# rlangefe/pygemma

Hardware: AMD Instinct MI355X
Metric: SNPs/sec (whole node) at n=10,000 c=5; K-eigendecomp wallclock (higher is better)
Workload: dtype i8x3->i32 MFMA (genotype codes exact, integer accumulation exact; U as 24-bit fixed point per eigenvector in three int8 planes) rotation + f64 Gram/sweeps (f32 rounding points of the reference)

## Files before the change

### include/pygemma_hip.h

```cpp
#ifndef PYGEMMA_HIP_H
#define PYGEMMA_HIP_H
#include <stddef.h>
#include <stdint.h>
#ifdef __cplusplus
extern "C" {
#endif

#define PG_OK 0
#define PG_EINVAL (-22)
#define PG_ENOMEM (-12)
#define PG_EHIP (-5)
#define PG_ENOTSUP (-95)
#define PG_ENODEV (-19)

#define PG_MAX_COVARIATES 30

typedef struct pg_ctx pg_ctx;

const char *pg_last_error(void);
const char *pg_version(void);
int pg_device_count(void);
int pg_ctx_create(int device, pg_ctx **out);
int pg_ctx_create_on_stream(int device, void *hip_stream, pg_ctx **out);
void pg_ctx_destroy(pg_ctx *ctx);
// ... 33 lines not shown
int pg_comm_destroy(pg_comm *comm);
int pg_comm_size(const pg_comm *comm);
int pg_comm_rank(const pg_comm *comm);
int pg_comm_broadcast_dev(pg_comm *comm, void *buf, size_t bytes, int root);
int pg_comm_allgather_dev(pg_comm *comm, const void *send, void *recv, size_t bytes_per_rank);
int pg_comm_allreduce_f64_dev(pg_comm *comm, double *buf, size_t count, int op_max);
int pg_comm_barrier(pg_comm *comm);
int pg_comm_group_start(void);
int pg_comm_group_end(void);

int pg_assoc_dev(pg_ctx *ctx, int64_t n, int c, int64_t p, const float *d, const float *Wr, const float *yr,
                 const float *Xr, int64_t ldx, int grid, float *beta, float *se, float *tau, float *lambda,
                 double *F, double *pval, unsigned long long *stats_dev);

int pg_assoc_set_eval_trace(pg_ctx *ctx, unsigned *trace_dev);
int pg_assoc_warm(pg_ctx *ctx, int64_t n, int c);

int pg_assoc_pheno_dev(pg_ctx *ctx, int64_t n, int c, int64_t p, int t, const float *d, const float *Wr,
                       const float *Yr, int64_t ldy, const float *Xr, int64_t ldx, int grid,
                       float *beta, float *se, float *tau, float *lambda, double *F, double *pval,
                       unsigned long long *stats_dev);
int pg_assoc_pheno_warm(pg_ctx *ctx, int64_t n, int c, int t, int64_t p);

int pg_assoc_lrt_dev(pg_ctx *ctx, int64_t n, int c, int64_t p, const float *d, const float *Wr, const float *yr,
                     const float *Xr, int64_t ldx, int grid, float *beta, float *se, float *tau, float *lambda,
                     double *F, double *pval, double *l_alt, double *l_null, double *D_lrt, double *p_lrt);

int pg_score_null_dev(pg_ctx *ctx, int64_t n, int c, const float *d, const float *Wr, const float *yr, float *lambda0_dev);
int pg_score_dev(pg_ctx *ctx, int64_t n, int c, int64_t p, const float *d, const float *Wr, const float *yr, float lambda0,
                 const float *Xr, int64_t ldx, float *beta, float *se, float *tau, float *lambda, double *F, double *pval);
// ... 78 lines not shown
```

### pygemma_amd/csrc/assoc.hip

```cpp
#include "common.hpp"

#include <cmath>

namespace pg {

constexpr int NLAM = 11;
#ifndef PG_ASSOC_WPB
#define PG_ASSOC_WPB 2
#endif
constexpr int WPB = PG_ASSOC_WPB;
#define PG_MINV 1e-35f
#ifndef PG_FUSE_PQ_MAX
#define PG_FUSE_PQ_MAX 36
#endif
#ifndef PG_FUSE_PQR_MAX
#define PG_FUSE_PQR_MAX 28
#endif
#ifndef PG_PFD
#define PG_PFD 2
#endif
#ifndef PG_CHUNK_MIN_NP
#define PG_CHUNK_MIN_NP 80
#endif
#ifndef PG_SCAN_NV
#define PG_SCAN_NV 96
#endif
#ifndef PG_SWEEP_LDS_MIN_SLOTS
#define PG_SWEEP_LDS_MIN_SLOTS 3
#endif
#ifndef PG_PHENO_SPLIT_XE
#define PG_PHENO_SPLIT_XE 26
#endif
#ifndef PG_WAVES
#define PG_WAVES 2
#endif

__host__ __device__ constexpr size_t assoc_per_wave_bytes(int M, bool sweep_lds, size_t evalout_bytes, int n_vals)
{
    return (((sweep_lds ? (size_t)3 * M * 8 : 0) + (size_t)NLAM * 2 * M * 8 + NLAM * evalout_bytes + 2 * NLAM * 4 + (size_t)n_vals * 4) + 15) & ~(size_t)15;
}

struct AssocParams {
    int n, npad, c, niter, nu, grid, rowf;
    long long p, ldx;
    const float *xr;
    const float *fixed;
    float *htab;
    double *fixg;
    double *t1tab;
    float *ldHtab;
    float lam11[NLAM];
    float logl_c;
    const int *leaf, *node, *level, *chunk;
    int n_leaf, n_level, n_chunk, n_vals;
    float *beta, *se, *tau, *lam;
    double *F;
    unsigned long long *stats;
    unsigned *trace;
    int lrt, nhalf;
    float ml_c;
    float *lalt, *lamalt;
    const double *xbuf;
    int xe, xcol;
};

struct EvalOut { float yPy, yPPy, yPPPy, trP, trPP, ld, Pxx_c, Pyx_c, sh, shh; };

__device__ __forceinline__ float hinv_f32(float lam, float d)
{
    const float x = __fadd_rn(__fmul_rn(lam, d), 1.0f);
    const float r0 = __builtin_amdgcn_rcpf(x);
    float r = __builtin_fmaf(__builtin_fmaf(-x, r0, 1.0f), r0, r0);
    if (__builtin_expect(!(x < 0x1p126f), 0)) r = __fdiv_rn(1.0f, x);
// ... 135 lines not shown
    r = (float)((double)r - ((0.5 * (double)pr.n) * ((2.0 * (double)G2) - (double)__fdiv_rn(__fmul_rn(G1, G1), a))) / (double)a);
    return r;
}

template <int C> struct Shape {
    static constexpr int M = C + 2;
    static constexpr int NP = M * (M + 1) / 2;
    static constexpr int SLOTS = (NP + 63) / 64;
    static constexpr int NV0 = NP < 64 ? NP : 64, NV1 = NP > 64 ? NP - 64 : 0;
    static constexpr int slot_nv(int sl) { return (NP - 64 * sl) < 64 ? (NP - 64 * sl) : 64; }
    static constexpr bool CHUNKED = NP > PG_CHUNK_MIN_NP;
    static constexpr bool SWEEP_LDS = SLOTS >= PG_SWEEP_LDS_MIN_SLOTS;
    static constexpr int SCAN_NV = (M <= 4 && PG_SCAN_NV > 64) ? 64 : PG_SCAN_NV;
    static constexpr int G = (SCAN_NV / (2 * M)) < 1 ? 1 : ((SCAN_NV / (2 * M)) > 11 ? 11 : (SCAN_NV / (2 * M)));
    static constexpr bool FUSE_PQ = NP <= PG_FUSE_PQ_MAX, FUSE_PQR = NP <= PG_FUSE_PQR_MAX;
};
__host__ __device__ constexpr int tri(int r, int c) { return r * (r + 1) / 2 + c; }
__host__ __device__ constexpr int next_pow2(int v) { int p = 1; while (p < v) p <<= 1; return p; }

__device__ __forceinline__ double dmaxf(double a, float b) { return ((double)b > a) ? (double)b : a; }

template <int NVP>
__device__ __forceinline__ double reduce_scatter(double (&v)[NVP], int lane)
{
    static_assert(NVP >= 1 && NVP <= 64 && (NVP & (NVP - 1)) == 0, "power of two");
#pragma unroll
    for (int s = 1; s < NVP; s <<= 1) {
        const bool b = (lane & s) != 0;
#pragma unroll
        for (int m = 0; m < NVP / (2 * s); m++) {
            const double keep = b ? v[2 * m + 1] : v[2 * m];
// ... 34 lines not shown
        }
    }
};

template <int SLOTS>
__device__ __forceinline__ double gather(const double (&X)[SLOTS], int es)
{
    double v = __shfl(X[0], es & 63, 64);
#pragma unroll
    for (int sl = 1; sl < SLOTS; sl++) { const double w = __shfl(X[sl], es & 63, 64); v = ((es >> 6) == sl) ? w : v; }
    return v;
}

__device__ __forceinline__ void wave_lds_sync();

template <int C, bool FULL>
__device__ __forceinline__ void lane_sweeps(double (&P)[Shape<C>::SLOTS], double (&Q)[Shape<C>::SLOTS], double (&R)[Shape<C>::SLOTS],
                                            const Own<C> &own, double t1, double t2, int lane, EvalOut &o, double *piv)
{
    constexpr int M = Shape<C>::M, NP = Shape<C>::NP, SLOTS = Shape<C>::SLOTS;
    constexpr bool VIA_LDS = Shape<C>::SWEEP_LDS;
    if (own.valid[0] && own.e[0] == 0) P[0] = dmaxf(P[0], PG_MINV);
    double trP = t1, trPP = t2, apiv = 1.0;
    for (int i = 1; i < M; i++) {
        const int q = i - 1, eqq = tri(q, q);
        double a, b, e = 0.0;
        double ur[SLOTS], uc[SLOTS], vr[SLOTS], vc[SLOTS], wr[SLOTS], wc[SLOTS];
        bool act[SLOTS];
        if constexpr (VIA_LDS) {
#pragma unroll
            for (int sl = 0; sl < SLOTS; sl++)
                if (own.valid[sl] && own.c[sl] == q) {
                    piv[own.r[sl]] = P[sl]; piv[M + own.r[sl]] = Q[sl];
                    if (FULL) piv[2 * M + own.r[sl]] = R[sl];
                }
            wave_lds_sync();
            a = piv[q]; b = piv[M + q];
            if (FULL) e = piv[2 * M + q];
#pragma unroll
            for (int sl = 0; sl < SLOTS; sl++) {
                act[sl] = own.valid[sl] && own.c[sl] >= i;
                const int rr = act[sl] ? own.r[sl] : q, cc = act[sl] ? own.c[sl] : q;
                ur[sl] = piv[rr]; uc[sl] = piv[cc];
                vr[sl] = piv[M + rr]; vc[sl] = piv[M + cc];
                if (FULL) { wr[sl] = piv[2 * M + rr]; wc[sl] = piv[2 * M + cc]; }
            }
            wave_lds_sync();
        } else {
            a = gather<SLOTS>(P, eqq); b = gather<SLOTS>(Q, eqq);
            e = FULL ? gather<SLOTS>(R, eqq) : 0.0;
#pragma unroll
            for (int sl = 0; sl < SLOTS; sl++) {
                act[sl] = own.valid[sl] && own.c[sl] >= i;
                const int er = act[sl] ? tri(own.r[sl], q) : 0, ec = act[sl] ? tri(own.c[sl], q) : 0;
                ur[sl] = gather<SLOTS>(P, er); uc[sl] = gather<SLOTS>(P, ec);
                vr[sl] = gather<SLOTS>(Q, er); vc[sl] = gather<SLOTS>(Q, ec);
                if (FULL) { wr[sl] = gather<SLOTS>(R, er); wc[sl] = gather<SLOTS>(R, ec); }
            }
        }
        if (lane == q) apiv = a;
        const double a2 = a * a, ia = -1.0 / a, ba2 = b / a2;
        if (FULL) {
            const double ba = b / a;
            trPP = (trPP + ba * ba) - 2 * (e / a);
            const double a3 = a2 * a, b2 = b * b;
            const double cR = (e / a2) - (b2 / a3);
#pragma unroll
            for (int sl = 0; sl < SLOTS; sl++)
                if (act[sl]) {
                    double s1 = fma(cR * uc[sl], ur[sl], R[sl]);
                    double s2 = fma(ia * uc[sl], wr[sl], 0.0); s2 = fma(ia * wc[sl], ur[sl], s2);
                    double s3 = fma(ia * vc[sl], vr[sl], 0.0);
                    double s4 = fma(ba2 * uc[sl], vr[sl], 0.0); s4 = fma(ba2 * vc[sl], ur[sl], s4);
                    double rn = ((s1 + s2) + s3) + s4;
                    if (own.r[sl] == i && own.c[sl] == i) rn = dmaxf(rn, PG_MINV);
                    R[sl] = rn;
                }
        }
        trP = trP - b / a;
#pragma unroll
        for (int sl = 0; sl < SLOTS; sl++)
            if (act[sl]) {
                double s1 = fma(ba2 * uc[sl], ur[sl], Q[sl]);
                double s2 = fma(ia * uc[sl], vr[sl], 0.0); s2 = fma(ia * vc[sl], ur[sl], s2);
                double qn = s1 + s2;
                double pn = fma(ia * uc[sl], ur[sl], P[sl]);
                if (own.r[sl] == i && own.c[sl] == i) { qn = dmaxf(qn, PG_MINV); pn = dmaxf(pn, PG_MINV); }
                Q[sl] = qn; P[sl] = pn;
            }
        if (i == M - 2) { o.Pxx_c = (float)gather<SLOTS>(P, tri(M - 2, M - 2)); o.Pyx_c = (float)gather<SLOTS>(P, tri(M - 1, M - 2)); }
    }
    const double lg = log(apiv);
    float ld = 0.0f;
    for (int q = 0; q < M - 1; q++) ld = (float)((double)ld + __shfl(lg, q, 64));
    o.yPy = (float)gather<SLOTS>(P, NP - 1);
    o.yPPy = (float)gather<SLOTS>(Q, NP - 1);
    o.yPPPy = FULL ? (float)gather<SLOTS>(R, NP - 1) : 0.0f;
    o.trP = (float)trP;
    o.trPP = FULL ? (float)trPP : 0.0f;
    o.ld = ld;
    o.sh = (float)t1;
    o.shh = FULL ? (float)t2 : 0.0f;
}

template <int C> struct Elem {
    static constexpr int S4 = (C + 2 + 3) / 4;
    float4 row[S4];
    float x;
};
template <int C, bool HASX = true>
__device__ __forceinline__ void load_elem(const AssocParams &pr, const float *xrow, int i, Elem<C> &e)
{
    const float4 *src = reinterpret_cast<const float4 *>(pr.fixed + (size_t)i * pr.rowf);
// ... 122 lines not shown
            }
        if constexpr (SL == 0 && PW == 1) s += hd;
        if constexpr (SL == 0 && PW == 3) s = fma(hd, hd, s);
    });
    out = reduce_scatter<NVP>(acc, lane);
    if constexpr (SL == 0 && (PW == 1 || PW == 3)) tsum = bfly(s);
}
template <int C, int PW, bool HASX, int SL = 0, class EL = WaldElem<C>>
__device__ __forceinline__ void slot_passes(const AssocParams &pr, typename EL::Row xrow, float lam, int lane, float *htab_out,
                                            double (&X)[Shape<C>::SLOTS], double &tsum)
{
    gram_pass_slot<C, PW, SL, HASX, EL>(pr, xrow, lam, lane, SL == 0 ? htab_out : nullptr, X[SL], tsum);
    if constexpr (SL + 1 < Shape<C>::SLOTS) slot_passes<C, PW, HASX, SL + 1, EL>(pr, xrow, lam, lane, htab_out, X, tsum);
}

template <int C, bool FULL, class EL = WaldElem<C>>
__device__ __forceinline__ void eval_specific(const AssocParams &pr, typename EL::Row xrow, float lam, int lane, const Own<C> &own, EvalOut &o,
                                              double *piv)
{
    constexpr int SLOTS = Shape<C>::SLOTS;
    double P[SLOTS], Q[SLOTS], R[SLOTS], t1 = 0.0, t2 = 0.0;
#pragma unroll
    for (int sl = 0; sl < SLOTS; sl++) R[sl] = 0.0;
    if constexpr (Shape<C>::CHUNKED) {
        double tq = 0.0;
        slot_passes<C, 1, true, 0, EL>(pr, xrow, lam, lane, nullptr, P, t1);
        slot_passes<C, 2, true, 0, EL>(pr, xrow, lam, lane, nullptr, Q, tq);
        if (FULL) slot_passes<C, 3, true, 0, EL>(pr, xrow, lam, lane, nullptr, R, t2);
    } else if constexpr (FULL && Shape<C>::FUSE_PQR) {
        gram_pass<C, 7, true, EL>(pr, xrow, lam, lane, nullptr, P, Q, R, t1, t2);
    } else if constexpr (Shape<C>::FUSE_PQ) {
        gram_pass<C, 3, true, EL>(pr, xrow, lam, lane, nullptr, P, Q, R, t1, t2);
        if (FULL) gram_pass<C, 4, true, EL>(pr, xrow, lam, lane, nullptr, P, Q, R, t1, t2);
    } else {
        gram_pass<C, 1, true, EL>(pr, xrow, lam, lane, nullptr, P, Q, R, t1, t2);
        gram_pass<C, 2, true, EL>(pr, xrow, lam, lane, nullptr, P, Q, R, t1, t2);
        if (FULL) gram_pass<C, 4, true, EL>(pr, xrow, lam, lane, nullptr, P, Q, R, t1, t2);
    }
    lane_sweeps<C, FULL>(P, Q, R, own, t1, t2, lane, o, piv);
}

template <int C>
__global__ __launch_bounds__(64) void setup_tabs_kernel(AssocParams pr)
{
    constexpr int NP = Shape<C>::NP, SLOTS = Shape<C>::SLOTS;
    extern __shared__ float smem_f[];
    const int t = blockIdx.x, lane = threadIdx.x;
    const float lam = pr.lam11[t];
    Own<C> own;
    own.init(lane);
    double P[SLOTS], Q[SLOTS], R[SLOTS], t1 = 0.0, t2 = 0.0;
    if constexpr (Shape<C>::CHUNKED) {
        double tq = 0.0;
        slot_passes<C, 1, false>(pr, nullptr, lam, lane, pr.htab + (size_t)t * pr.npad, P, t1);
// ... 236 lines not shown
        iteration++;
    }
    return lroot;
}

template <int C, bool LRT, bool PHENO = false>
__global__ __launch_bounds__(64 * WPB, PG_WAVES) void assoc_kernel(AssocParams pr)
{
    constexpr int M = Shape<C>::M, NP = Shape<C>::NP, SLOTS = Shape<C>::SLOTS;
    extern __shared__ unsigned char smem[];
    const int wave = threadIdx.x >> 6, lane = threadIdx.x & 63;
    static_assert(!(PHENO && LRT), "the multi-phenotype search has no LRT");
    const long long g = (long long)blockIdx.x * WPB + wave;
    if (g >= pr.p) return;
    constexpr size_t piv_bytes = Shape<C>::SWEEP_LDS ? (size_t)3 * M * 8 : 0;
    unsigned char *base = smem + (size_t)wave * assoc_per_wave_bytes(M, Shape<C>::SWEEP_LDS, sizeof(EvalOut), pr.n_vals);
    double *piv = reinterpret_cast<double *>(base);
    base += piv_bytes;
    double *xent = reinterpret_cast<double *>(base);
    EvalOut *evs = reinterpret_cast<EvalOut *>(base + (size_t)NLAM * 2 * M * 8);
    float *d1s = reinterpret_cast<float *>(evs + NLAM);
    float *lls = d1s + NLAM;
    float *vals = lls + NLAM;
    const float *xrow = pr.xr + (size_t)g * pr.ldx;

    Own<C> own;
    own.init(lane);
    if constexpr (PHENO) {
        const double *src = pr.xbuf + (size_t)g * NLAM * 2 * pr.xe;
        for (int j = lane; j < NLAM * 2 * M; j += 64) {
            const int tp = j / M, k = j - tp * M;
            xent[j] = src[(size_t)tp * pr.xe + (k <= C ? k : pr.xcol)];
        }
// ... 3 lines not shown
    wave_lds_sync();
    for (int t = 0; t < NLAM; t++) {
        double P[SLOTS], Q[SLOTS], R[SLOTS];
        const double *fp = pr.fixg + ((size_t)t * 2 + 0) * NP, *fq = pr.fixg + ((size_t)t * 2 + 1) * NP;
        const double *xe = xent + t * 2 * M;
#pragma unroll
        for (int sl = 0; sl < SLOTS; sl++) {
            const int r = own.r[sl], c = own.c[sl];
            const bool isx = (r == C) || (r == C + 1 && c == C);
            const int k = (r == C) ? c : C + 1;
            P[sl] = isx ? xe[k] : fp[own.e[sl]];
            Q[sl] = isx ? xe[M + k] : fq[own.e[sl]];
            R[sl] = 0.0;
        }
        EvalOut e;
        lane_sweeps<C, false>(P, Q, R, own, pr.t1tab[t], 0.0, lane, e, piv);
        if (lane == 0) {
            evs[t] = e;
            d1s[t] = d1_f(pr, pr.lam11[t], e.yPy, e.yPPy, e.trP);
            lls[t] = logl_f(pr, e.yPy, pr.ldHtab[t], e.ld);
        }
    }
    wave_lds_sync();
    float best_l = lls[0], best_lambda;
    EvalOut best_e;
    if (best_l < lls[NLAM - 1]) { best_l = lls[NLAM - 1]; best_lambda = pr.lam11[NLAM - 1]; best_e = evs[NLAM - 1]; }
    else { best_lambda = pr.lam11[0]; best_e = evs[0]; }
    unsigned n_fast = 0, n_full = 0;
    if (pr.grid) {
        for (int t = 0; t < NLAM - 1; t++)
            if (lls[t] > best_l) { best_l = lls[t]; best_lambda = pr.lam11[t]; best_e = evs[t]; }
    } else {
        for (int k = 0; k < NLAM - 1; k++) {
            const float f0 = d1s[k], f1 = d1s[k + 1];
            if (__builtin_signbit(f0) == __builtin_signbit(f1)) continue;
            const float l0 = pr.lam11[k], l1 = pr.lam11[k + 1];
            double root = brentq_dev(
                [&](double x) -> double {
                    EvalOut e;
                    const float lf = (float)x;
                    eval_specific<C, false>(pr, xrow, lf, lane, own, e, piv);
                    n_fast++;
                    return (double)d1_f(pr, lf, e.yPy, e.yPPy, e.trP);
                },
                (double)l0, (double)l1, (double)f0, (double)f1);
            const float lroot = newton_dev(pr, (float)root, l0, l1, [&](float lf, EvalOut &e) {
                eval_specific<C, true>(pr, xrow, lf, lane, own, e, piv);
                n_full++;
            });
            EvalOut e;
            eval_specific<C, false>(pr, xrow, lroot, lane, own, e, piv);
            n_fast++;
            const float ldH = device_logdet_H(pr, lroot, lane, vals);
            const float ll = logl_f(pr, e.yPy, ldH, e.ld);
            if (ll > best_l) { best_l = ll; best_lambda = lroot; best_e = e; }
        }
    }
    if constexpr (LRT) {
        float ml_l = ml_logl_f(pr, evs[0].yPy, pr.ldHtab[0]), ml_lam = pr.lam11[0];
        {
            const float l1 = ml_logl_f(pr, evs[NLAM - 1].yPy, pr.ldHtab[NLAM - 1]);
            if (ml_l == ml_l && (l1 != l1 || l1 > ml_l)) { ml_l = l1; ml_lam = pr.lam11[NLAM - 1]; }
        }
        for (int k = 0; k < NLAM - 1; k++) {
            const float f0 = ml_d1_f(pr, pr.lam11[k], evs[k].yPy, evs[k].yPPy, evs[k].sh);
            const float f1 = ml_d1_f(pr, pr.lam11[k + 1], evs[k + 1].yPy, evs[k + 1].yPPy, evs[k + 1].sh);
            if (f0 != f0 || f1 != f1) continue;
            const float s0 = (float)((f0 > 0) - (f0 < 0)), s1 = (float)((f1 > 0) - (f1 < 0));
            if (!(s0 * s1 < 0.0f)) continue;
            double p0 = brentq_dev(
                [&](double x) -> double {
                    EvalOut e;
                    const float lf = (float)x;
                    eval_specific<C, false>(pr, xrow, lf, lane, own, e, piv);
                    n_fast++;
                    return (double)ml_d1_f(pr, lf, e.yPy, e.yPPy, e.sh);
                },
                (double)pr.lam11[k], (double)pr.lam11[k + 1], (double)f0, (double)f1, 5000);
            double pn = p0;
            for (int itr = 0; itr < 10; itr++) {
                EvalOut e;
                const float lf = (float)p0;
                eval_specific<C, true>(pr, xrow, lf, lane, own, e, piv);
                n_full++;
                const float fval = ml_d1_f(pr, lf, e.yPy, e.yPPy, e.sh);
                if (fval == 0.0f) { pn = p0; break; }
                const float fder = ml_d2_f(pr, lf, e.yPy, e.yPPy, e.yPPPy, e.sh, e.shh);
                if (fder == 0.0f) { pn = p0; break; }
                pn = p0 - (double)__fdiv_rn(fval, fder);
                if (fabs(pn - p0) <= 1.48e-8 + 1e-5 * fabs(p0)) break;
                p0 = pn;
            }
            if (ml_l == ml_l) {
                EvalOut e;
                const float lf = (float)pn;
                eval_specific<C, false>(pr, xrow, lf, lane, own, e, piv);
                n_fast++;
                const float l = ml_logl_f(pr, e.yPy, device_logdet_H(pr, lf, lane, vals));
                if (l != l || l > ml_l) { ml_l = l; ml_lam = lf; }
            }
        }
        if (lane == 0) { pr.lalt[g] = ml_l; pr.lamalt[g] = ml_lam; }
    }
    if (lane == 0) {
        const float b = __fdiv_rn(best_e.Pyx_c, best_e.Pxx_c);
        const float pxx = (PG_MINV > best_e.Pxx_c) ? PG_MINV : best_e.Pxx_c;
        const float sb = (float)(__dsqrt_rn((double)best_e.yPy) / ((double)sqrtf(pxx) * __dsqrt_rn((double)(pr.nu))));
        const float ta = __fdiv_rn((float)pr.nu, best_e.yPy);
        const double t = (double)__fdiv_rn(b, sb);
        pr.beta[g] = b; pr.se[g] = sb; pr.tau[g] = ta; pr.lam[g] = best_lambda; pr.F[g] = t * t;
        if (pr.stats) { atomicAdd(&pr.stats[0], (unsigned long long)n_fast); atomicAdd(&pr.stats[1], (unsigned long long)n_full); }
        if (pr.trace) pr.trace[g] = n_fast | (n_full << 16);
    }
}

#if defined(PG_ASSOC_PART) && (PG_ASSOC_PART == 6 || PG_ASSOC_PART == 7)
struct GxeRows { const float *x, *xe; };
template <int CS> struct GxeVals {
    static constexpr int S4 = (CS + 2 + 3) / 4;
    float4 row[S4];
    float x, xe;
};
template <int C> struct GxeElem {
    static constexpr int CS = C - 1;
    using E = GxeVals<CS>;
    using Row = GxeRows;
    template <bool HASX>
// ... 137 lines not shown
    for (int t = 0; t < NLAM; t++) {
        double P[SLOTS], Q[SLOTS], R[SLOTS];
        const double *fp = pr.fixg + ((size_t)t * 2 + 0) * NPS, *fq = pr.fixg + ((size_t)t * 2 + 1) * NPS;
        const double *xe = xent + t * 2 * NE;
#pragma unroll
        for (int sl = 0; sl < SLOTS; sl++) {
            const int r = own.r[sl], c = own.c[sl];
            const int k = (r == CS) ? c : (r == CS + 1) ? CS + 1 + c : (r == CS + 2 && c == CS) ? 2 * CS + 3 : (r == CS + 2 && c == CS + 1) ? 2 * CS + 4 : -1;
            const int f = (r < CS) ? tri(r, c) : tri(CS + 1, c < CS ? c : CS + 1);
            const int kk = k >= 0 ? k : 0;
            P[sl] = k >= 0 ? xe[kk] : fp[f];
            Q[sl] = k >= 0 ? xe[NE + kk] : fq[f];
            R[sl] = 0.0;
        }
        EvalOut e;
        lane_sweeps<C, false>(P, Q, R, own, pr.t1tab[t], 0.0, lane, e, piv);
        if (lane == 0) {
            evs[t] = e;
            d1s[t] = d1_f(pr, pr.lam11[t], e.yPy, e.yPPy, e.trP);
            lls[t] = logl_f(pr, e.yPy, pr.ldHtab[t], e.ld);
        }
    }
    wave_lds_sync();
    float best_l = lls[0], best_lambda;
    EvalOut best_e;
    if (best_l < lls[NLAM - 1]) { best_l = lls[NLAM - 1]; best_lambda = pr.lam11[NLAM - 1]; best_e = evs[NLAM - 1]; }
    else { best_lambda = pr.lam11[0]; best_e = evs[0]; }
    unsigned n_fast = 0, n_full = 0;
    for (int k = 0; k < NLAM - 1; k++) {
        const float f0 = d1s[k], f1 = d1s[k + 1];
        if (__builtin_signbit(f0) == __builtin_signbit(f1)) continue;
        const float l0 = pr.lam11[k], l1 = pr.lam11[k + 1];
        double root = brentq_dev(
            [&](double x) -> double {
                EvalOut e;
                const float lf = (float)x;
                eval_specific<C, false, EL>(pr, xr, lf, lane, own, e, piv);
                n_fast++;
                return (double)d1_f(pr, lf, e.yPy, e.yPPy, e.trP);
            },
            (double)l0, (double)l1, (double)f0, (double)f1);
        const float lroot = newton_dev(pr, (float)root, l0, l1, [&](float lf, EvalOut &e) {
            eval_specific<C, true, EL>(pr, xr, lf, lane, own, e, piv);
            n_full++;
        });
        EvalOut e;
        eval_specific<C, false, EL>(pr, xr, lroot, lane, own, e, piv);
        n_fast++;
        const float ldH = device_logdet_H(pr, lroot, lane, vals);
        const float ll = logl_f(pr, e.yPy, ldH, e.ld);
        if (ll > best_l) { best_l = ll; best_lambda = lroot; best_e = e; }
    }
    if (lane == 0) {
        const float b = __fdiv_rn(best_e.Pyx_c, best_e.Pxx_c);
        const float pxx = (PG_MINV > best_e.Pxx_c) ? PG_MINV : best_e.Pxx_c;
        const float sb = (float)(__dsqrt_rn((double)best_e.yPy) / ((double)sqrtf(pxx) * __dsqrt_rn((double)(pr.nu))));
        const float ta = __fdiv_rn((float)pr.nu, best_e.yPy);
        const double t = (double)__fdiv_rn(b, sb);
        pr.beta[g] = b; pr.se[g] = sb; pr.tau[g] = ta; pr.lam[g] = best_lambda; pr.F[g] = t * t;
        if (pr.stats) { atomicAdd(&pr.stats[0], (unsigned long long)n_fast); atomicAdd(&pr.stats[1], (unsigned long long)n_full); }
    }
}
// ... 6 lines not shown
    PG_REQUIRE(pr.n_vals >= 0 && lds <= 160 * 1024, "assoc_gxe: c = %d, n_vals = %d need %zu bytes of LDS per workgroup", CS, pr.n_vals, lds);
    setup_tabs_kernel<CS><<<NLAM, 64, (size_t)pr.n_vals * 4 + 16, ctx->stream>>>(pr);
    PG_HIP(hipGetLastError());
    if (lds > 64 * 1024)
        PG_HIP(hipFuncSetAttribute(reinterpret_cast<const void *>(&assoc_gxe_kernel<CS>), hipFuncAttributeMaxDynamicSharedMemorySize, (int)lds));
    const long long nblk = (pr.p + WPB - 1) / WPB;
    assoc_gxe_kernel<CS><<<dim3((unsigned)nblk), 64 * WPB, lds, ctx->stream>>>(pr, xer, ldxe);
    PG_HIP(hipGetLastError());
    return PG_OK;
}
#endif

template <int C, bool LRT = false>
static int launch_assoc(pg_ctx *ctx, AssocParams &pr)
{
    const size_t lds = (size_t)WPB * assoc_per_wave_bytes(Shape<C>::M, Shape<C>::SWEEP_LDS, sizeof(EvalOut), pr.n_vals);
    static_assert(Shape<C>::M == C + 2, "Shape<C>::M");
    PG_REQUIRE(pr.n_vals >= 0 && lds <= 160 * 1024, "assoc: c = %d, n_vals = %d need %zu bytes of LDS per workgroup", C, pr.n_vals, lds);
    setup_tabs_kernel<C><<<NLAM, 64, (size_t)pr.n_vals * 4 + 16, ctx->stream>>>(pr);
    PG_HIP(hipGetLastError());
    if (lds > 64 * 1024)
        PG_HIP(hipFuncSetAttribute(reinterpret_cast<const void *>(&assoc_kernel<C, LRT>), hipFuncAttributeMaxDynamicSharedMemorySize, (int)lds));
    const long long nblk = (pr.p + WPB - 1) / WPB;
    assoc_kernel<C, LRT><<<dim3((unsigned)nblk), 64 * WPB, lds, ctx->stream>>>(pr);
    PG_HIP(hipGetLastError());
    return PG_OK;
}

struct PhenoLaunch {
    enum { SETUP, SCAN, SEARCH } phase;
    const float *Y; long long ldy;
// ... 4 lines not shown
template <int C>
static int launch_pheno(pg_ctx *ctx, AssocParams &pr, const PhenoLaunch &pl)
{
    if (pl.phase == PhenoLaunch::SETUP) {
        setup_tabs_kernel<C><<<NLAM, 64, (size_t)pr.n_vals * 4 + 16, ctx->stream>>>(pr);
    } else if (pl.phase == PhenoLaunch::SCAN) {
        const unsigned nblk = (unsigned)((pr.p + SCAN_WPB - 1) / SCAN_WPB);
        switch (pl.tpad) {
            case 1: scan_pheno_kernel<C, 1><<<nblk, 64 * SCAN_WPB, 0, ctx->stream>>>(pr, pl.Y, pl.ldy, pl.tcn, pl.xbuf); break;
            case 2: scan_pheno_kernel<C, 2><<<nblk, 64 * SCAN_WPB, 0, ctx->stream>>>(pr, pl.Y, pl.ldy, pl.tcn, pl.xbuf); break;
            case 4: scan_pheno_kernel<C, 4><<<nblk, 64 * SCAN_WPB, 0, ctx->stream>>>(pr, pl.Y, pl.ldy, pl.tcn, pl.xbuf); break;
            case 8: scan_pheno_kernel<C, 8><<<nblk, 64 * SCAN_WPB, 0, ctx->stream>>>(pr, pl.Y, pl.ldy, pl.tcn, pl.xbuf); break;
            default: set_error("assoc_pheno: chunk width %d", pl.tpad); return PG_EINVAL;
        }
    } else {
        const size_t lds = (size_t)WPB * assoc_per_wave_bytes(Shape<C>::M, Shape<C>::SWEEP_LDS, sizeof(EvalOut), pr.n_vals);
        PG_REQUIRE(pr.n_vals >= 0 && lds <= 160 * 1024, "assoc_pheno: c = %d, n_vals = %d need %zu bytes of LDS per workgroup", C, pr.n_vals, lds);
        if (lds > 64 * 1024)
            PG_HIP(hipFuncSetAttribute(reinterpret_cast<const void *>(&assoc_kernel<C, false, true>), hipFuncAttributeMaxDynamicSharedMemorySize, (int)lds));
        const long long nblk = (pr.p + WPB - 1) / WPB;
        assoc_kernel<C, false, true><<<dim3((unsigned)nblk), 64 * WPB, lds, ctx->stream>>>(pr);
    }
    PG_HIP(hipGetLastError());
    return PG_OK;
}


int launch_assoc_hi(pg_ctx *ctx, AssocParams &pr);
int launch_assoc_lrt(pg_ctx *ctx, AssocParams &pr);
int launch_assoc_lrt_hi(pg_ctx *ctx, AssocParams &pr);
int launch_assoc_pheno(pg_ctx *ctx, AssocParams &pr, const PhenoLaunch &pl);
// ... 413 lines not shown
    const size_t off_t1 = off_fixg + (size_t)NLAM * 2 * NP * 8;
    const size_t off_ldh = off_t1 + NLAM * 8;
    rc = ensure(ctx, &ctx->tabs, &ctx->tabs_bytes, off_ldh + NLAM * 4 + 256);
    if (rc) return rc;
    if (!ctx->stats) PG_HIP(hipMalloc(&ctx->stats, 16));
    pr.fixed = (const float *)ctx->fixed;
    pr.htab = (float *)ctx->tabs;
    pr.fixg = (double *)((char *)ctx->tabs + off_fixg);
    pr.t1tab = (double *)((char *)ctx->tabs + off_t1);
    pr.ldHtab = (float *)((char *)ctx->tabs + off_ldh);
    pr.lrt = lrt ? 1 : 0;
    pr.lalt = lalt; pr.lamalt = lamalt;
    pr.beta = beta; pr.se = se; pr.tau = tau; pr.lam = lambda; pr.F = F;
    pr.stats = stats_dev;
    pr.trace = lrt ? nullptr : ctx->eval_trace;

    build_fixed_kernel<<<(pr.npad + 255) / 256, 256, 0, ctx->stream>>>(pr.n, pr.npad, c, (int)ldw, pr.rowf, d, Wr, yr, (float *)ctx->fixed);
    PG_HIP(hipGetLastError());
    return launch_assoc_any(ctx, pr);
}

extern "C" int pg_assoc_dev(pg_ctx *ctx, int64_t n, int c, int64_t p, const float *d, const float *Wr, const float *yr,
                            const float *Xr, int64_t ldx, int grid, float *beta, float *se, float *tau, float *lambda,
                            double *F, double *pval, unsigned long long *stats_dev)
{
    PG_REQUIRE(ctx && d && Wr && yr && Xr && beta && se && tau && lambda && F, "pg_assoc_dev: NULL argument");
    PG_REQUIRE(n >= 2 && n < (1LL << 30) && p >= 0 && ldx >= n, "pg_assoc_dev: bad shape n=%lld p=%lld ldx=%lld", (long long)n, (long long)p, (long long)ldx);
    if (c < 1 || c > PG_MAX_COVARIATES) {
        set_error("pg_assoc_dev: c=%d covariates not supported by this build (1..%d)", c, PG_MAX_COVARIATES);
        return PG_ENOTSUP;
// ... 18 lines not shown
    if (rc) return rc;
    const int npad = (int)((n + 63) / 64 * 64), rowf = ((c + 2 + 3) / 4) * 4, M = c + 2, NP = M * (M + 1) / 2;
    rc = ensure(ctx, &ctx->fixed, &ctx->fixed_bytes, (size_t)npad * rowf * 4);
    if (rc) return rc;
    const size_t off_fixg = ((size_t)NLAM * npad * 4 + 255) & ~(size_t)255;
    rc = ensure(ctx, &ctx->tabs, &ctx->tabs_bytes, off_fixg + (size_t)NLAM * 2 * NP * 8 + NLAM * 8 + NLAM * 4 + 256);
    if (rc) return rc;
    if (!ctx->stats) PG_HIP(hipMalloc(&ctx->stats, 16));
    return PG_OK;
}

extern "C" int pg_assoc_set_eval_trace(pg_ctx *ctx, unsigned *trace_dev)
{
    PG_REQUIRE(ctx, "pg_assoc_set_eval_trace: NULL ctx");
    ctx->eval_trace = trace_dev;
    return PG_OK;
}

struct PhenoLayout {
    int npad, rowf, NP, tpad_max;
    long long ptile;
    size_t off_htab, off_fixg, off_t1, off_ldh, off_xbuf, bytes;
};
static PhenoLayout pheno_layout(int64_t n, int c, int t, int64_t p)
{
    PhenoLayout L{};
    auto up = [](size_t v) { return (v + 255) & ~(size_t)255; };
    L.npad = (int)((n + 63) / 64 * 64); L.rowf = ((c + 2 + 3) / 4) * 4; L.NP = (c + 2) * (c + 3) / 2;
    const int tc = t < PHENO_CHUNK ? t : PHENO_CHUNK;
    L.tpad_max = 1;
// ... 313 lines not shown
```

### pygemma_amd/csrc/common.hpp

```cpp
#pragma once
#include <hip/hip_runtime.h>
#include <cstdarg>
#include <cstdint>
#include <cstdio>
#include <cstring>
#include <vector>

#include "../../include/pygemma_hip.h"

namespace pg {

void set_error(const char *fmt, ...);

#define PG_HIP(call)                                                                             \
    do {                                                                                         \
        hipError_t _e = (call);                                                                  \
        if (_e != hipSuccess) {                                                                  \
            pg::set_error("%s failed: %s (%s:%d)", #call, hipGetErrorString(_e), __FILE__, __LINE__); \
            return PG_EHIP;                                                                      \
        }                                                                                        \
    } while (0)

#define PG_REQUIRE(cond, ...)            \
    do {                                 \
// ... 11 lines not shown
    int *d_level = nullptr;
    int *d_chunk = nullptr;
};

}

struct pg_ctx {
    int device = 0;
    hipStream_t stream = nullptr;
    bool own_stream = true;
    int num_cu = 256;
    void *fixed = nullptr; size_t fixed_bytes = 0;
    void *tabs = nullptr;  size_t tabs_bytes = 0;
    unsigned long long *stats = nullptr;
    unsigned *eval_trace = nullptr;
    pg::NpSumPlan plan;
    void *pheno = nullptr; size_t pheno_bytes = 0;
    void *score = nullptr; size_t score_bytes = 0;
    void *scratch = nullptr; size_t scratch_bytes = 0;
    void *arena = nullptr; size_t arena_bytes = 0;
    void *hpin = nullptr; size_t hpin_bytes = 0;
};

namespace pg {
int ensure(pg_ctx *ctx, void **ptr, size_t *have, size_t need);
int build_npsum_plan(pg_ctx *ctx, int64_t n);
}
```

### pygemma_amd/ops.py

```python
import ctypes as C

import numpy as np

from . import _lib


def _f32(a):
    return np.ascontiguousarray(a, dtype=np.float32)


def assoc(d, Wr, yr, Xr, grid=False, ctx=None, want_p=True, return_stats=False):
    L = _lib.load()
    with _lib.scope(ctx) as ctx:
        d, Wr, yr, Xr = _f32(d), _f32(Wr), _f32(np.asarray(yr).reshape(-1)), _f32(Xr)
        n, c = Wr.shape
        p = Xr.shape[1]
        assert d.shape == (n,) and yr.shape == (n,) and Xr.shape[0] == n
        beta, se, tau, lam = (np.empty(p, np.float32) for _ in range(4))
        F, pv = np.empty(p, np.float64), np.empty(p, np.float64)
        stats = np.zeros(2, np.uint64)
        vp = lambda a: a.ctypes.data_as(C.c_void_p)
        _lib.check(L.pg_assoc(ctx.handle, n, c, p, vp(d), vp(Wr), vp(yr), vp(Xr), int(bool(grid)), vp(beta), vp(se),
                              vp(tau), vp(lam), vp(F), vp(pv) if want_p else None, vp(stats)), "pg_assoc")
        out = {"beta": beta, "se_beta": se, "tau": tau, "lambda": lam.astype(np.float64), "F_wald": F,
               "p_wald": pv if want_p else None}
        if return_stats:
            out["n_evals"] = stats.astype(np.int64)
        return out


def score(d, Wr, yr, Xr, lam0=None, ctx=None):
    L = _lib.load()
    with _lib.scope(ctx) as ctx:
        d, Wr, yr, Xr = _f32(d), _f32(Wr), _f32(np.asarray(yr).reshape(-1)), _f32(Xr)
        n, c = Wr.shape
        p = Xr.shape[1]
        assert d.shape == (n,) and yr.shape == (n,) and Xr.shape[0] == n
        dd, dW, dy = ctx.to_device(d), ctx.to_device(Wr), ctx.to_device(yr)
        if lam0 is None:
            dl = ctx.alloc(4)
            _lib.check(L.pg_score_null_dev(ctx.handle, n, c, dd.ptr, dW.ptr, dy.ptr, dl.ptr), "pg_score_null_dev")
            ctx.sync()
# ... 122 lines not shown
```

Before: 1.760 million.

## Reuse Brent P/Q Gram passes in Newton and compute only P at final eval

Generalizes the per-lambda Gram/sweep evaluation to a power mask so the final post-Newton evaluation computes only the P matrix, skipping the Q Gram pass and Q sweeps, since only yPy and logdet are used there. During Brent iterations the last two P/Q Gram results are saved in LDS per lane. If the first Newton step hits one of those lambdas bit-exactly, only the R pass is computed. This adds LDS per wave, which may reduce occupancy, and adds optional pass-count statistics.

```diff
diff --git a/include/pygemma_hip.h b/include/pygemma_hip.h
--- a/include/pygemma_hip.h
+++ b/include/pygemma_hip.h
@@ -71,6 +71,7 @@
                  double *F, double *pval, unsigned long long *stats_dev);
 
 int pg_assoc_set_eval_trace(pg_ctx *ctx, unsigned *trace_dev);
+int pg_assoc_set_pass_stats(pg_ctx *ctx, unsigned long long *dev4);
 int pg_assoc_warm(pg_ctx *ctx, int64_t n, int c);
 
 int pg_assoc_pheno_dev(pg_ctx *ctx, int64_t n, int c, int64_t p, int t, const float *d, const float *Wr,
diff --git a/pygemma_amd/csrc/assoc.hip b/pygemma_amd/csrc/assoc.hip
--- a/pygemma_amd/csrc/assoc.hip
+++ b/pygemma_amd/csrc/assoc.hip
@@ -34,10 +34,21 @@
 #ifndef PG_WAVES
 #define PG_WAVES 2
 #endif
-
-__host__ __device__ constexpr size_t assoc_per_wave_bytes(int M, bool sweep_lds, size_t evalout_bytes, int n_vals)
-{
-    return (((sweep_lds ? (size_t)3 * M * 8 : 0) + (size_t)NLAM * 2 * M * 8 + NLAM * evalout_bytes + 2 * NLAM * 4 + (size_t)n_vals * 4) + 15) & ~(size_t)15;
+#ifndef PG_ASSOC_FINAL_P
+#define PG_ASSOC_FINAL_P 1
+#endif
+#ifndef PG_ASSOC_NEWTON_REUSE
+#define PG_ASSOC_NEWTON_REUSE 1
+#endif
+#ifndef PG_REUSE_MAX_SLOTS
+#define PG_REUSE_MAX_SLOTS 4
+#endif
+
+__host__ __device__ constexpr size_t assoc_sav_doubles(int sav_slots) { return sav_slots ? (size_t)2 * (2 * sav_slots + 1) * 64 : 0; }
+__host__ __device__ constexpr size_t assoc_per_wave_bytes(int M, bool sweep_lds, int sav_slots, size_t evalout_bytes, int n_vals)
+{
+    return (((sweep_lds ? (size_t)3 * M * 8 : 0) + assoc_sav_doubles(sav_slots) * 8 + (size_t)NLAM * 2 * M * 8 + NLAM * evalout_bytes + 2 * NLAM * 4 +
+             (size_t)n_vals * 4) + 15) & ~(size_t)15;
 }
 
 struct AssocParams {
@@ -57,6 +68,7 @@
     double *F;
     unsigned long long *stats;
     unsigned *trace;
+    unsigned long long *passes;
     int lrt, nhalf;
     float ml_c;
     float *lalt, *lamalt;
@@ -222,7 +234,10 @@
     static constexpr int SCAN_NV = (M <= 4 && PG_SCAN_NV > 64) ? 64 : PG_SCAN_NV;
     static constexpr int G = (SCAN_NV / (2 * M)) < 1 ? 1 : ((SCAN_NV / (2 * M)) > 11 ? 11 : (SCAN_NV / (2 * M)));
     static constexpr bool FUSE_PQ = NP <= PG_FUSE_PQ_MAX, FUSE_PQR = NP <= PG_FUSE_PQR_MAX;
+    static constexpr bool NEWTON_REUSE = PG_ASSOC_NEWTON_REUSE && SLOTS <= PG_REUSE_MAX_SLOTS;
+    static constexpr int SAV_SLOTS = NEWTON_REUSE ? SLOTS : 0, SAV_STRIDE = (2 * SLOTS + 1) * 64;
 };
+constexpr int PW_P = 1, PW_PQ = 3, PW_R = 4, PW_PQR = 7;
 __host__ __device__ constexpr int tri(int r, int c) { return r * (r + 1) / 2 + c; }
 __host__ __device__ constexpr int next_pow2(int v) { int p = 1; while (p < v) p <<= 1; return p; }
 
@@ -287,53 +302,58 @@
 
 __device__ __forceinline__ void wave_lds_sync();
 
-template <int C, bool FULL>
+template <int C, int PW>
 __device__ __forceinline__ void lane_sweeps(double (&P)[Shape<C>::SLOTS], double (&Q)[Shape<C>::SLOTS], double (&R)[Shape<C>::SLOTS],
                                             const Own<C> &own, double t1, double t2, int lane, EvalOut &o, double *piv)
 {
     constexpr int M = Shape<C>::M, NP = Shape<C>::NP, SLOTS = Shape<C>::SLOTS;
+    static_assert(PW == PW_P || PW == PW_PQ || PW == PW_PQR, "powers");
+    constexpr bool DQ = (PW & 2) != 0, FULL = (PW & 4) != 0;
     constexpr bool VIA_LDS = Shape<C>::SWEEP_LDS;
     if (own.valid[0] && own.e[0] == 0) P[0] = dmaxf(P[0], PG_MINV);
     double trP = t1, trPP = t2, apiv = 1.0;
     for (int i = 1; i < M; i++) {
         const int q = i - 1, eqq = tri(q, q);
-        double a, b, e = 0.0;
+        double a, b = 0.0, e = 0.0;
         double ur[SLOTS], uc[SLOTS], vr[SLOTS], vc[SLOTS], wr[SLOTS], wc[SLOTS];
         bool act[SLOTS];
         if constexpr (VIA_LDS) {
 #pragma unroll
             for (int sl = 0; sl < SLOTS; sl++)
                 if (own.valid[sl] && own.c[sl] == q) {
-                    piv[own.r[sl]] = P[sl]; piv[M + own.r[sl]] = Q[sl];
+                    piv[own.r[sl]] = P[sl];
+                    if (DQ) piv[M + own.r[sl]] = Q[sl];
                     if (FULL) piv[2 * M + own.r[sl]] = R[sl];
                 }
             wave_lds_sync();
-            a = piv[q]; b = piv[M + q];
+            a = piv[q];
+            if (DQ) b = piv[M + q];
             if (FULL) e = piv[2 * M + q];
 #pragma unroll
             for (int sl = 0; sl < SLOTS; sl++) {
                 act[sl] = own.valid[sl] && own.c[sl] >= i;
                 const int rr = act[sl] ? own.r[sl] : q, cc = act[sl] ? own.c[sl] : q;
                 ur[sl] = piv[rr]; uc[sl] = piv[cc];
-                vr[sl] = piv[M + rr]; vc[sl] = piv[M + cc];
+                if (DQ) { vr[sl] = piv[M + rr]; vc[sl] = piv[M + cc]; }
                 if (FULL) { wr[sl] = piv[2 * M + rr]; wc[sl] = piv[2 * M + cc]; }
             }
             wave_lds_sync();
         } else {
-            a = gather<SLOTS>(P, eqq); b = gather<SLOTS>(Q, eqq);
-            e = FULL ? gather<SLOTS>(R, eqq) : 0.0;
+            a = gather<SLOTS>(P, eqq);
+            if (DQ) b = gather<SLOTS>(Q, eqq);
+            if (FULL) e = gather<SLOTS>(R, eqq);
 #pragma unroll
             for (int sl = 0; sl < SLOTS; sl++) {
                 act[sl] = own.valid[sl] && own.c[sl] >= i;
                 const int er = act[sl] ? tri(own.r[sl], q) : 0, ec = act[sl] ? tri(own.c[sl], q) : 0;
                 ur[sl] = gather<SLOTS>(P, er); uc[sl] = gather<SLOTS>(P, ec);
-                vr[sl] = gather<SLOTS>(Q, er); vc[sl] = gather<SLOTS>(Q, ec);
+                if (DQ) { vr[sl] = gather<SLOTS>(Q, er); vc[sl] = gather<SLOTS>(Q, ec); }
                 if (FULL) { wr[sl] = gather<SLOTS>(R, er); wc[sl] = gather<SLOTS>(R, ec); }
             }
         }
         if (lane == q) apiv = a;
         const double a2 = a * a, ia = -1.0 / a, ba2 = b / a2;
-        if (FULL) {
+        if constexpr (FULL) {
             const double ba = b / a;
             trPP = (trPP + ba * ba) - 2 * (e / a);
             const double a3 = a2 * a, b2 = b * b;
@@ -350,26 +370,36 @@
                     R[sl] = rn;
                 }
         }
-        trP = trP - b / a;
-#pragma unroll
-        for (int sl = 0; sl < SLOTS; sl++)
-            if (act[sl]) {
-                double s1 = fma(ba2 * uc[sl], ur[sl], Q[sl]);
-                double s2 = fma(ia * uc[sl], vr[sl], 0.0); s2 = fma(ia * vc[sl], ur[sl], s2);
-                double qn = s1 + s2;
-                double pn = fma(ia * uc[sl], ur[sl], P[sl]);
-                if (own.r[sl] == i && own.c[sl] == i) { qn = dmaxf(qn, PG_MINV); pn = dmaxf(pn, PG_MINV); }
-                Q[sl] = qn; P[sl] = pn;
-            }
+        if constexpr (DQ) {
+            trP = trP - b / a;
+#pragma unroll
+            for (int sl = 0; sl < SLOTS; sl++)
+                if (act[sl]) {
+                    double s1 = fma(ba2 * uc[sl], ur[sl], Q[sl]);
+                    double s2 = fma(ia * uc[sl], vr[sl], 0.0); s2 = fma(ia * vc[sl], ur[sl], s2);
+                    double qn = s1 + s2;
+                    double pn = fma(ia * uc[sl], ur[sl], P[sl]);
+                    if (own.r[sl] == i && own.c[sl] == i) { qn = dmaxf(qn, PG_MINV); pn = dmaxf(pn, PG_MINV); }
+                    Q[sl] = qn; P[sl] = pn;
+                }
+        } else {
+#pragma unroll
+            for (int sl = 0; sl < SLOTS; sl++)
+                if (act[sl]) {
+                    double pn = fma(ia * uc[sl], ur[sl], P[sl]);
+                    if (own.r[sl] == i && own.c[sl] == i) pn = dmaxf(pn, PG_MINV);
+                    P[sl] = pn;
+                }
+        }
         if (i == M - 2) { o.Pxx_c = (float)gather<SLOTS>(P, tri(M - 2, M - 2)); o.Pyx_c = (float)gather<SLOTS>(P, tri(M - 1, M - 2)); }
     }
     const double lg = log(apiv);
     float ld = 0.0f;
     for (int q = 0; q < M - 1; q++) ld = (float)((double)ld + __shfl(lg, q, 64));
     o.yPy = (float)gather<SLOTS>(P, NP - 1);
-    o.yPPy = (float)gather<SLOTS>(Q, NP - 1);
+    o.yPPy = DQ ? (float)gather<SLOTS>(Q, NP - 1) : 0.0f;
     o.yPPPy = FULL ? (float)gather<SLOTS>(R, NP - 1) : 0.0f;
-    o.trP = (float)trP;
+    o.trP = DQ ? (float)trP : 0.0f;
     o.trPP = FULL ? (float)trPP : 0.0f;
     o.ld = ld;
     o.sh = (float)t1;
@@ -522,30 +552,39 @@
     if constexpr (SL + 1 < Shape<C>::SLOTS) slot_passes<C, PW, HASX, SL + 1, EL>(pr, xrow, lam, lane, htab_out, X, tsum);
 }
 
-template <int C, bool FULL, class EL = WaldElem<C>>
+template <int C, int MASK, class EL = WaldElem<C>>
+__device__ __forceinline__ void gram_powers(const AssocParams &pr, typename EL::Row xrow, float lam, int lane,
+                                            double (&P)[Shape<C>::SLOTS], double (&Q)[Shape<C>::SLOTS], double (&R)[Shape<C>::SLOTS],
+                                            double &t1, double &t2)
+{
+    constexpr bool DP = (MASK & 1) != 0, DQ = (MASK & 2) != 0, DR = (MASK & 4) != 0;
+    if constexpr (Shape<C>::CHUNKED) {
+        double tq = 0.0;
+        if constexpr (DP) slot_passes<C, 1, true, 0, EL>(pr, xrow, lam, lane, nullptr, P, t1);
+        if constexpr (DQ) slot_passes<C, 2, true, 0, EL>(pr, xrow, lam, lane, nullptr, Q, tq);
+        if constexpr (DR) slot_passes<C, 3, true, 0, EL>(pr, xrow, lam, lane, nullptr, R, t2);
+    } else if constexpr (MASK == PW_PQR && Shape<C>::FUSE_PQR) {
+        gram_pass<C, 7, true, EL>(pr, xrow, lam, lane, nullptr, P, Q, R, t1, t2);
+    } else if constexpr (DP && DQ && Shape<C>::FUSE_PQ) {
+        gram_pass<C, 3, true, EL>(pr, xrow, lam, lane, nullptr, P, Q, R, t1, t2);
+        if constexpr (DR) gram_pass<C, 4, true, EL>(pr, xrow, lam, lane, nullptr, P, Q, R, t1, t2);
+    } else {
+        if constexpr (DP) gram_pass<C, 1, true, EL>(pr, xrow, lam, lane, nullptr, P, Q, R, t1, t2);
+        if constexpr (DQ) gram_pass<C, 2, true, EL>(pr, xrow, lam, lane, nullptr, P, Q, R, t1, t2);
+        if constexpr (DR) gram_pass<C, 4, true, EL>(pr, xrow, lam, lane, nullptr, P, Q, R, t1, t2);
+    }
+}
+
+template <int C, int PW, class EL = WaldElem<C>>
 __device__ __forceinline__ void eval_specific(const AssocParams &pr, typename EL::Row xrow, float lam, int lane, const Own<C> &own, EvalOut &o,
                                               double *piv)
 {
     constexpr int SLOTS = Shape<C>::SLOTS;
     double P[SLOTS], Q[SLOTS], R[SLOTS], t1 = 0.0, t2 = 0.0;
 #pragma unroll
-    for (int sl = 0; sl < SLOTS; sl++) R[sl] = 0.0;
-    if constexpr (Shape<C>::CHUNKED) {
-        double tq = 0.0;
-        slot_passes<C, 1, true, 0, EL>(pr, xrow, lam, lane, nullptr, P, t1);
-        slot_passes<C, 2, true, 0, EL>(pr, xrow, lam, lane, nullptr, Q, tq);
-        if (FULL) slot_passes<C, 3, true, 0, EL>(pr, xrow, lam, lane, nullptr, R, t2);
-    } else if constexpr (FULL && Shape<C>::FUSE_PQR) {
-        gram_pass<C, 7, true, EL>(pr, xrow, lam, lane, nullptr, P, Q, R, t1, t2);
-    } else if constexpr (Shape<C>::FUSE_PQ) {
-        gram_pass<C, 3, true, EL>(pr, xrow, lam, lane, nullptr, P, Q, R, t1, t2);
-        if (FULL) gram_pass<C, 4, true, EL>(pr, xrow, lam, lane, nullptr, P, Q, R, t1, t2);
-    } else {
-        gram_pass<C, 1, true, EL>(pr, xrow, lam, lane, nullptr, P, Q, R, t1, t2);
-        gram_pass<C, 2, true, EL>(pr, xrow, lam, lane, nullptr, P, Q, R, t1, t2);
-        if (FULL) gram_pass<C, 4, true, EL>(pr, xrow, lam, lane, nullptr, P, Q, R, t1, t2);
-    }
-    lane_sweeps<C, FULL>(P, Q, R, own, t1, t2, lane, o, piv);
+    for (int sl = 0; sl < SLOTS; sl++) { Q[sl] = 0.0; R[sl] = 0.0; }
+    gram_powers<C, PW, EL>(pr, xrow, lam, lane, P, Q, R, t1, t2);
+    lane_sweeps<C, PW>(P, Q, R, own, t1, t2, lane, o, piv);
 }
 
 template <int C>
@@ -812,9 +851,12 @@
     const long long g = (long long)blockIdx.x * WPB + wave;
     if (g >= pr.p) return;
     constexpr size_t piv_bytes = Shape<C>::SWEEP_LDS ? (size_t)3 * M * 8 : 0;
-    unsigned char *base = smem + (size_t)wave * assoc_per_wave_bytes(M, Shape<C>::SWEEP_LDS, sizeof(EvalOut), pr.n_vals);
+    constexpr bool REUSE = Shape<C>::NEWTON_REUSE;
+    unsigned char *base = smem + (size_t)wave * assoc_per_wave_bytes(M, Shape<C>::SWEEP_LDS, Shape<C>::SAV_SLOTS, sizeof(EvalOut), pr.n_vals);
     double *piv = reinterpret_cast<double *>(base);
     base += piv_bytes;
+    double *sav = reinterpret_cast<double *>(base) + lane;
+    base += assoc_sav_doubles(Shape<C>::SAV_SLOTS) * 8;
     double *xent = reinterpret_cast<double *>(base);
     EvalOut *evs = reinterpret_cast<EvalOut *>(base + (size_t)NLAM * 2 * M * 8);
     float *d1s = reinterpret_cast<float *>(evs + NLAM);
@@ -848,7 +890,7 @@
             R[sl] = 0.0;
         }
         EvalOut e;
-        lane_sweeps<C, false>(P, Q, R, own, pr.t1tab[t], 0.0, lane, e, piv);
+        lane_sweeps<C, PW_PQ>(P, Q, R, own, pr.t1tab[t], 0.0, lane, e, piv);
         if (lane == 0) {
             evs[t] = e;
             d1s[t] = d1_f(pr, pr.lam11[t], e.yPy, e.yPPy, e.trP);
@@ -860,7 +902,8 @@
     EvalOut best_e;
     if (best_l < lls[NLAM - 1]) { best_l = lls[NLAM - 1]; best_lambda = pr.lam11[NLAM - 1]; best_e = evs[NLAM - 1]; }
     else { best_lambda = pr.lam11[0]; best_e = evs[0]; }
-    unsigned n_fast = 0, n_full = 0;
+    unsigned n_fast = 0, n_full = 0, n_ponly = 0, n_reuse = 0;
+    constexpr int PW_FINAL = PG_ASSOC_FINAL_P ? PW_P : PW_PQ;
     if (pr.grid) {
         for (int t = 0; t < NLAM - 1; t++)
             if (lls[t] > best_l) { best_l = lls[t]; best_lambda = pr.lam11[t]; best_e = evs[t]; }
@@ -869,22 +912,58 @@
             const float f0 = d1s[k], f1 = d1s[k + 1];
             if (__builtin_signbit(f0) == __builtin_signbit(f1)) continue;
             const float l0 = pr.lam11[k], l1 = pr.lam11[k + 1];
+            float sav_lam0 = NAN, sav_lam1 = NAN;
+            unsigned sav_next = 0;
             double root = brentq_dev(
                 [&](double x) -> double {
                     EvalOut e;
                     const float lf = (float)x;
-                    eval_specific<C, false>(pr, xrow, lf, lane, own, e, piv);
+                    if constexpr (REUSE) {
+                        double P[SLOTS], Q[SLOTS], R[SLOTS], t1 = 0.0, t2 = 0.0;
+#pragma unroll
+                        for (int sl = 0; sl < SLOTS; sl++) R[sl] = 0.0;
+                        gram_powers<C, PW_PQ>(pr, xrow, lf, lane, P, Q, R, t1, t2);
+                        double *sv = sav + sav_next * Shape<C>::SAV_STRIDE;
+#pragma unroll
+                        for (int sl = 0; sl < SLOTS; sl++) { sv[64 * sl] = P[sl]; sv[64 * (SLOTS + sl)] = Q[sl]; }
+                        sv[64 * 2 * SLOTS] = t1;
+                        if (sav_next) sav_lam1 = lf; else sav_lam0 = lf;
+                        sav_next ^= 1u;
+                        lane_sweeps<C, PW_PQ>(P, Q, R, own, t1, t2, lane, e, piv);
+                    } else {
+                        eval_specific<C, PW_PQ>(pr, xrow, lf, lane, own, e, piv);
+                    }
                     n_fast++;
                     return (double)d1_f(pr, lf, e.yPy, e.yPPy, e.trP);
                 },
                 (double)l0, (double)l1, (double)f0, (double)f1);
+            bool first = true;
             const float lroot = newton_dev(pr, (float)root, l0, l1, [&](float lf, EvalOut &e) {
-                eval_specific<C, true>(pr, xrow, lf, lane, own, e, piv);
+                if constexpr (REUSE) {
+                    const unsigned lb = __float_as_uint(lf);
+                    const int hit = !(first && lf == lf) ? -1 : (lb == __float_as_uint(sav_lam0)) ? 0 : (lb == __float_as_uint(sav_lam1)) ? 1 : -1;
+                    first = false;
+                    double P[SLOTS], Q[SLOTS], R[SLOTS], t1 = 0.0, t2 = 0.0;
+                    if (hit >= 0) {
+                        const double *sv = sav + hit * Shape<C>::SAV_STRIDE;
+#pragma unroll
+                        for (int sl = 0; sl < SLOTS; sl++) { P[sl] = sv[64 * sl]; Q[sl] = sv[64 * (SLOTS + sl)]; }
+                        t1 = sv[64 * 2 * SLOTS];
+                        gram_powers<C, PW_R>(pr, xrow, lf, lane, P, Q, R, t1, t2);
+                        n_reuse++;
+                    } else {
+                        gram_powers<C, PW_PQR>(pr, xrow, lf, lane, P, Q, R, t1, t2);
+                    }
+                    lane_sweeps<C, PW_PQR>(P, Q, R, own, t1, t2, lane, e, piv);
+                } else {
+                    eval_specific<C, PW_PQR>(pr, xrow, lf, lane, own, e, piv);
+                }
                 n_full++;
             });
             EvalOut e;
-            eval_specific<C, false>(pr, xrow, lroot, lane, own, e, piv);
+            eval_specific<C, PW_FINAL>(pr, xrow, lroot, lane, own, e, piv);
             n_fast++;
+            if (PW_FINAL == PW_P) n_ponly++;
             const float ldH = device_logdet_H(pr, lroot, lane, vals);
             const float ll = logl_f(pr, e.yPy, ldH, e.ld);
             if (ll > best_l) { best_l = ll; best_lambda = lroot; best_e = e; }
@@ -906,7 +985,7 @@
                 [&](double x) -> double {
                     EvalOut e;
                     const float lf = (float)x;
-                    eval_specific<C, false>(pr, xrow, lf, lane, own, e, piv);
+                    eval_specific<C, PW_PQ>(pr, xrow, lf, lane, own, e, piv);
                     n_fast++;
                     return (double)ml_d1_f(pr, lf, e.yPy, e.yPPy, e.sh);
                 },
@@ -915,7 +994,7 @@
             for (int itr = 0; itr < 10; itr++) {
                 EvalOut e;
                 const float lf = (float)p0;
-                eval_specific<C, true>(pr, xrow, lf, lane, own, e, piv);
+                eval_specific<C, PW_PQR>(pr, xrow, lf, lane, own, e, piv);
                 n_full++;
                 const float fval = ml_d1_f(pr, lf, e.yPy, e.yPPy, e.sh);
                 if (fval == 0.0f) { pn = p0; break; }
@@ -928,8 +1007,9 @@
             if (ml_l == ml_l) {
                 EvalOut e;
                 const float lf = (float)pn;
-                eval_specific<C, false>(pr, xrow, lf, lane, own, e, piv);
+                eval_specific<C, PW_FINAL>(pr, xrow, lf, lane, own, e, piv);
                 n_fast++;
+                if (PW_FINAL == PW_P) n_ponly++;
                 const float l = ml_logl_f(pr, e.yPy, device_logdet_H(pr, lf, lane, vals));
                 if (l != l || l > ml_l) { ml_l = l; ml_lam = lf; }
             }
@@ -945,6 +1025,11 @@
         pr.beta[g] = b; pr.se[g] = sb; pr.tau[g] = ta; pr.lam[g] = best_lambda; pr.F[g] = t * t;
         if (pr.stats) { atomicAdd(&pr.stats[0], (unsigned long long)n_fast); atomicAdd(&pr.stats[1], (unsigned long long)n_full); }
         if (pr.trace) pr.trace[g] = n_fast | (n_full << 16);
+        if (pr.passes) {
+            const unsigned long long np = (unsigned long long)(n_fast + n_full - n_reuse);
+            atomicAdd(&pr.passes[0], np); atomicAdd(&pr.passes[1], np - n_ponly);
+            atomicAdd(&pr.passes[2], (unsigned long long)n_full); atomicAdd(&pr.passes[3], (unsigned long long)n_reuse);
+        }
     }
 }
 
@@ -1112,7 +1197,7 @@
             R[sl] = 0.0;
         }
         EvalOut e;
-        lane_sweeps<C, false>(P, Q, R, own, pr.t1tab[t], 0.0, lane, e, piv);
+        lane_sweeps<C, PW_PQ>(P, Q, R, own, pr.t1tab[t], 0.0, lane, e, piv);
         if (lane == 0) {
             evs[t] = e;
             d1s[t] = d1_f(pr, pr.lam11[t], e.yPy, e.yPPy, e.trP);
@@ -1133,17 +1218,17 @@
             [&](double x) -> double {
                 EvalOut e;
                 const float lf = (float)x;
-                eval_specific<C, false, EL>(pr, xr, lf, lane, own, e, piv);
+                eval_specific<C, PW_PQ, EL>(pr, xr, lf, lane, own, e, piv);
                 n_fast++;
                 return (double)d1_f(pr, lf, e.yPy, e.yPPy, e.trP);
             },
             (double)l0, (double)l1, (double)f0, (double)f1);
         const float lroot = newton_dev(pr, (float)root, l0, l1, [&](float lf, EvalOut &e) {
-            eval_specific<C, true, EL>(pr, xr, lf, lane, own, e, piv);
+            eval_specific<C, PW_PQR, EL>(pr, xr, lf, lane, own, e, piv);
             n_full++;
         });
         EvalOut e;
-        eval_specific<C, false, EL>(pr, xr, lroot, lane, own, e, piv);
+        eval_specific<C, PW_PQ, EL>(pr, xr, lroot, lane, own, e, piv);
         n_fast++;
         const float ldH = device_logdet_H(pr, lroot, lane, vals);
         const float ll = logl_f(pr, e.yPy, ldH, e.ld);
@@ -1180,7 +1265,7 @@
 template <int C, bool LRT = false>
 static int launch_assoc(pg_ctx *ctx, AssocParams &pr)
 {
-    const size_t lds = (size_t)WPB * assoc_per_wave_bytes(Shape<C>::M, Shape<C>::SWEEP_LDS, sizeof(EvalOut), pr.n_vals);
+    const size_t lds = (size_t)WPB * assoc_per_wave_bytes(Shape<C>::M, Shape<C>::SWEEP_LDS, Shape<C>::SAV_SLOTS, sizeof(EvalOut), pr.n_vals);
     static_assert(Shape<C>::M == C + 2, "Shape<C>::M");
     PG_REQUIRE(pr.n_vals >= 0 && lds <= 160 * 1024, "assoc: c = %d, n_vals = %d need %zu bytes of LDS per workgroup", C, pr.n_vals, lds);
     setup_tabs_kernel<C><<<NLAM, 64, (size_t)pr.n_vals * 4 + 16, ctx->stream>>>(pr);
@@ -1215,7 +1300,7 @@
             default: set_error("assoc_pheno: chunk width %d", pl.tpad); return PG_EINVAL;
         }
     } else {
-        const size_t lds = (size_t)WPB * assoc_per_wave_bytes(Shape<C>::M, Shape<C>::SWEEP_LDS, sizeof(EvalOut), pr.n_vals);
+        const size_t lds = (size_t)WPB * assoc_per_wave_bytes(Shape<C>::M, Shape<C>::SWEEP_LDS, Shape<C>::SAV_SLOTS, sizeof(EvalOut), pr.n_vals);
         PG_REQUIRE(pr.n_vals >= 0 && lds <= 160 * 1024, "assoc_pheno: c = %d, n_vals = %d need %zu bytes of LDS per workgroup", C, pr.n_vals, lds);
         if (lds > 64 * 1024)
             PG_HIP(hipFuncSetAttribute(reinterpret_cast<const void *>(&assoc_kernel<C, false, true>), hipFuncAttributeMaxDynamicSharedMemorySize, (int)lds));
@@ -1659,6 +1744,7 @@
     pr.beta = beta; pr.se = se; pr.tau = tau; pr.lam = lambda; pr.F = F;
     pr.stats = stats_dev;
     pr.trace = lrt ? nullptr : ctx->eval_trace;
+    pr.passes = lrt ? nullptr : ctx->pass_stats;
 
     build_fixed_kernel<<<(pr.npad + 255) / 256, 256, 0, ctx->stream>>>(pr.n, pr.npad, c, (int)ldw, pr.rowf, d, Wr, yr, (float *)ctx->fixed);
     PG_HIP(hipGetLastError());
@@ -1707,6 +1793,13 @@
 {
     PG_REQUIRE(ctx, "pg_assoc_set_eval_trace: NULL ctx");
     ctx->eval_trace = trace_dev;
+    return PG_OK;
+}
+
+extern "C" int pg_assoc_set_pass_stats(pg_ctx *ctx, unsigned long long *dev4)
+{
+    PG_REQUIRE(ctx, "pg_assoc_set_pass_stats: NULL ctx");
+    ctx->pass_stats = dev4;
     return PG_OK;
 }
 
diff --git a/pygemma_amd/csrc/common.hpp b/pygemma_amd/csrc/common.hpp
--- a/pygemma_amd/csrc/common.hpp
+++ b/pygemma_amd/csrc/common.hpp
@@ -49,6 +49,7 @@
     void *tabs = nullptr;  size_t tabs_bytes = 0;
     unsigned long long *stats = nullptr;
     unsigned *eval_trace = nullptr;
+    unsigned long long *pass_stats = nullptr;
     pg::NpSumPlan plan;
     void *pheno = nullptr; size_t pheno_bytes = 0;
     void *score = nullptr; size_t score_bytes = 0;
diff --git a/pygemma_amd/ops.py b/pygemma_amd/ops.py
--- a/pygemma_amd/ops.py
+++ b/pygemma_amd/ops.py
@@ -20,12 +20,20 @@
         F, pv = np.empty(p, np.float64), np.empty(p, np.float64)
         stats = np.zeros(2, np.uint64)
         vp = lambda a: a.ctypes.data_as(C.c_void_p)
-        _lib.check(L.pg_assoc(ctx.handle, n, c, p, vp(d), vp(Wr), vp(yr), vp(Xr), int(bool(grid)), vp(beta), vp(se),
-                              vp(tau), vp(lam), vp(F), vp(pv) if want_p else None, vp(stats)), "pg_assoc")
+        dpass = ctx.to_device(np.zeros(4, np.uint64)) if return_stats else None
+        if return_stats:
+            _lib.check(L.pg_assoc_set_pass_stats(ctx.handle, dpass.ptr), "pg_assoc_set_pass_stats")
+        try:
+            _lib.check(L.pg_assoc(ctx.handle, n, c, p, vp(d), vp(Wr), vp(yr), vp(Xr), int(bool(grid)), vp(beta), vp(se),
+                                  vp(tau), vp(lam), vp(F), vp(pv) if want_p else None, vp(stats)), "pg_assoc")
+        finally:
+            if return_stats:
+                L.pg_assoc_set_pass_stats(ctx.handle, None)
         out = {"beta": beta, "se_beta": se, "tau": tau, "lambda": lam.astype(np.float64), "F_wald": F,
                "p_wald": pv if want_p else None}
         if return_stats:
             out["n_evals"] = stats.astype(np.int64)
+            out["passes"] = dpass.download((4,), np.uint64).astype(np.int64)
         return out
 
 
```

New measurement: 1.806 million (median of 6 runs). +2.6%, better.
